# nubot-nudt/LCR-Net

Measured on AMD Instinct MI355X. Metric: scans/s (120k-pt KITTI-shape scan -> 256-D descriptor), higher is better.
Workload: dtype f32 (K-deep GEMMs, K >= 288 and N >= 64: fp32 operands as bf16 x 3 split, 6 of 9 products on the bf16 matrix cores, fp32 accumulate — error vs fp64 <= the fp32-MFMA kernel's; every other GEMM, KPConv and attention: fp32 MFMA); 1 GPU; configs[1]: batch of 8 synthetic 64-beam scans (~120k pts, 0.3 m voxel -> ~16k pts), voxelise + 3 subsamples + 10 radius searches + KPConv encoder + NetVLAD, seeded random weights; distinct_input_batches=4, streams=pre-processing stream (own host thread, 2 batches ahead) + 2 encoder stream(s), parallelism=scan-parallel x1, all-gather of descriptors

## Files before the change

### include/lcr_hip.h

```cpp
#ifndef LCR_HIP_H
#define LCR_HIP_H
#include <stddef.h>
#include <stdint.h>
#ifdef __cplusplus
extern "C" {
#endif

#define LCR_OK 0
#define LCR_EARG (-1)
#define LCR_ESPACE (-2)
#define LCR_EHIP (-3)

#define LCR_STATUS_KEY_OVERFLOW 1u
#define LCR_STATUS_LEN_MISMATCH 2u
#define LCR_GN_REPLICAS 8

const char* lcr_last_error(void);
void lcr_ktimer_enable(int on);
void lcr_ktimer_sample(int every);
void lcr_ktimer_kinds(unsigned mask);
int lcr_ktimer_read(int kind, int max_records, double* seconds, int64_t* meta);
int lcr_ktimer_read2(int kind, int max_records, double* seconds, double* seconds_kernel, int64_t* meta);
int lcr_stream_spin(int microseconds, void* stream);
int lcr_version(void);
// ... 65 lines not shown
  size_t  off_neighbors[LCR_MAX_STAGES];
  size_t  off_subsampling[LCR_MAX_STAGES];
  size_t  off_upsampling[LCR_MAX_STAGES];
  size_t  out_bytes, ws_bytes;
} LcrPrecomputeLayout;
int lcr_precompute_layout(int64_t n0, int B, int num_stages, const int* limits, int upsampling, int64_t n_raw,
                          LcrPrecomputeLayout* layout);
int lcr_precompute_batch(const float* points0, const int64_t* lengths0, const LcrPrecomputeLayout* layout, float voxel_size,
                         float radius, float raw_voxel, int key_bits_hint, void* out, size_t out_bytes, void* ws, size_t ws_bytes,
                         int64_t* lengths_host, uint32_t* status_host, void* stream);
int lcr_precompute_batch_rows(const float* points0, int raw_row_floats, const int64_t* lengths0, const LcrPrecomputeLayout* layout,
                              float voxel_size, float radius, float raw_voxel, int key_bits_hint, void* out, size_t out_bytes, void* ws,
                              size_t ws_bytes, int64_t* lengths_host, uint32_t* status_host, void* stream);
int lcr_precompute_ws_bytes_ex(const LcrPrecomputeLayout* layout, int raw_method, size_t* bytes);
int lcr_precompute_batch_rows_ex(const float* points0, int raw_row_floats, const int64_t* lengths0, const LcrPrecomputeLayout* layout,
                                 float voxel_size, float radius, double raw_voxel, int raw_method, int key_bits_hint, void* out,
                                 size_t out_bytes, void* ws, size_t ws_bytes, int64_t* lengths_host, uint32_t* status_host, void* stream);

int lcr_gemm_f32(const float* A, const float* B, float* C, int64_t M, int N, int K, int transA, int transB,
                 const float* bias, const float* rowdiv, const int64_t* seg_len, int S, int groups, double* stats,
                 void* stream);
int lcr_split_bf16x3(const float* w, int64_t n, uint16_t* planes, void* stream);
int lcr_split_bf16x3_tiles(const float* w, int N, int K, uint16_t* tiles, void* stream);
int lcr_gemm_f32_bsplit(const float* A, const uint16_t* Bs_tiles, float* C, int64_t M, int N, int K, const float* bias, const float* rowdiv,
                        const int64_t* seg_len, int S, int groups, double* stats, void* stream);
int lcr_gemm_f32_masked(const float* A, const float* B, float* C, int64_t M, int N, int K, const float* bias, const float* rowdiv,
                        const int64_t* seg_len, int S, int groups, double* stats, const uint16_t* row_mask, int block_k, void* stream);
int lcr_gemm_f32_bsplit_masked(const float* A, const uint16_t* Bs_tiles, float* C, int64_t M, int N, int K, const float* bias,
                               const float* rowdiv, const int64_t* seg_len, int S, int groups, double* stats, const uint16_t* row_mask,
                               int block_k, void* stream);
int lcr_kpconv_mask_ok(int64_t M, int N, int K, int split);
int lcr_gemm_f32_anorm(const float* A, const float* B, float* C, int64_t M, int N, int K, const float* bias,
                       const double* a_stats, const float* a_gamma, const float* a_beta, int a_groups, float a_eps,
                       float a_slope, const int64_t* seg_len, int S, int groups, double* stats, void* stream);
int lcr_gemm_f32_bsplit_anorm(const float* A, const uint16_t* Bs_tiles, float* C, int64_t M, int N, int K, const float* bias,
                              const double* a_stats, const float* a_gamma, const float* a_beta, int a_groups, float a_eps,
                              float a_slope, const int64_t* seg_len, int S, int groups, double* stats, void* stream);
int lcr_gemm_split_ok(int N, int K);
int lcr_gemm_f32_batched_ta(const float* A, const float* B, float* C, int64_t M, int N, int count, const int* k_host,
                            const int64_t* a_off_host, const int64_t* b_off_host, const int64_t* c_off_host, void* stream);
int lcr_kpconv_aggregate(const float* s_feats, const uint8_t* s_pos, const float* q_pts, const float* s_pts,
                         const void* idx, int idx_is_64, int64_t M, int64_t Ns, int H, int C,
                         const float* kernel_points_host, float sigma, float* A, float* nn,
                         const int32_t* order , void* stream);
#define LCR_KP_VALID_FIRST 1
int lcr_kpconv_aggregate_ex(const float* s_feats, const uint8_t* s_pos, const float* q_pts, const float* s_pts,
                            const void* idx, int idx_is_64, int64_t M, int64_t Ns, int H, int C,
                            const float* kernel_points_host, float sigma, float* A, float* nn,
                            const int32_t* order, int flags, void* stream);
int lcr_kpconv_aggregate_mask(const float* s_feats, const uint8_t* s_pos, const float* q_pts, const float* s_pts,
                              const void* idx, int idx_is_64, int64_t M, int64_t Ns, int H, int C,
                              const float* kernel_points_host, float sigma, float* A, float* nn, uint16_t* mask,
                              const int32_t* order, int flags, void* stream);
int lcr_kpconv_fused(const float* s_feats, const uint8_t* s_pos, const float* q_pts, const float* s_pts, const void* idx,
                     int idx_is_64, int64_t M, int64_t Ns, int H, int C, const float* kernel_points_host, float sigma,
                     const float* W, const float* bias, float* out, const int64_t* seg_len, int S, int groups, double* stats,
                     const int32_t* order, void* stream);
int lcr_kpconv_cin1(const float* s_feats, const float* q_pts, const float* s_pts, const void* idx, int idx_is_64,
                    int64_t M, int64_t Ns, int H, const float* kernel_points_host, float sigma, const float* W,
                    const float* bias, int Cout, float* out, const int32_t* order, void* stream);
int lcr_maxpool(const float* x, const void* idx, int idx_is_64, int64_t M, int64_t Ns, int H, int C, float* out,
                const int32_t* order, void* stream);
int lcr_row_positive(const float* x, int64_t N, int C, uint8_t* pos, void* stream);
int lcr_groupnorm_stats(const float* x, int64_t N, int C, int groups, const int64_t* seg_len, int S, double* stats, void* stream);
int lcr_groupnorm_apply(const float* x, const double* stats, const float* gamma, const float* beta, const float* res,
                        const double* res_stats, const float* res_gamma, const float* res_beta, float* y, int64_t N, int C,
                        int groups, const int64_t* seg_len, int S, float eps, float slope, int act, uint8_t* pos, void* stream);

int lcr_neighbor_transpose_ws_bytes(int64_t M, int H, size_t* bytes);
int lcr_neighbor_transpose(const void* idx, int idx_is_64, int64_t M, int64_t Ns, int H, int32_t* row_start, uint32_t* edges,
                           void* ws, size_t ws_bytes, void* stream);
int lcr_kpconv_aggregate_grad(const float* dA, const float* q_pts, const float* s_pts, const int32_t* row_start, const uint32_t* edges,
                              int64_t M, int64_t Ns, int H, int C, const float* kernel_points_host, float sigma, float* d_s_feats,
                              void* stream);
int lcr_kpconv_cin1_grad_ws_bytes(int64_t M, int Cout, int want_feats, size_t* bytes);
int lcr_kpconv_cin1_grad(const float* d_out, const float* s_feats, const float* q_pts, const float* s_pts, const void* idx, int idx_is_64,
                         const float* nn, const int32_t* row_start, const uint32_t* edges, int64_t M, int64_t Ns, int H,
                         const float* kernel_points_host, float sigma, const float* W, int Cout, float* dW, float* dbias,
                         float* d_s_feats, void* ws, size_t ws_bytes, void* stream);
int lcr_maxpool_grad(const float* d_out, const float* x, const float* pooled, const void* idx, int idx_is_64, const int32_t* row_start,
                     const uint32_t* edges, int64_t M, int64_t Ns, int H, int C, uint8_t* winners, float* d_x, void* stream);
int lcr_kpconv_points_grad_ws_bytes(int64_t M, int H, size_t* bytes);
int lcr_kpconv_points_grad(const float* dA, const float* s_feats, const float* q_pts, const float* s_pts, const void* idx, int idx_is_64,
                           const int32_t* row_start, const uint32_t* edges, int64_t M, int64_t Ns, int H, int C,
                           const float* kernel_points_host, float sigma, float* d_q, float* d_s, void* ws, size_t ws_bytes, void* stream);
int lcr_groupnorm_apply_grad_ws_bytes(int64_t N, int C, int groups, int S, size_t* bytes);
int lcr_groupnorm_apply_grad(const float* x, const double* stats, const float* gamma, const float* y, const float* dy, int64_t N, int C,
                             int groups, const int64_t* seg_len, int S, float eps, float slope, int act, float* dx, float* dgamma,
                             float* dbeta, float* dz, void* ws, size_t ws_bytes, void* stream);

#define LCR_ENC_BLOCKS 10
typedef struct LcrUnaryW {
  const float *w, *b;
  const float *gn_w, *gn_b;
  const uint16_t* w_split;
} LcrUnaryW;
typedef struct LcrBlockW {
  int   cin, cout, strided;
  float sigma;
  const float* kernel_points_host;
  const float *kp_w, *kp_b;
  const float* kp_wt;
  const uint16_t* kp_wt_split;
  const float *normconv_w, *normconv_b;
  LcrUnaryW unary1, unary2, shortcut;
} LcrBlockW;
// ... 265 lines not shown
```

### include/lcr_hip_debug.h

```cpp
#ifndef LCR_HIP_DEBUG_H
#define LCR_HIP_DEBUG_H

#ifdef __cplusplus
extern "C" {
#endif

void lcr_gemm_debug_force_tile(int tile);
void lcr_gemm_debug_deep(int mode);
void lcr_gemm_debug_streamk(int mode);
void lcr_groupnorm_debug_general(int on);
void lcr_kpconv_debug_off64(int on);
void lcr_augment_debug_select_mask(uint32_t mask);

#ifdef __cplusplus
}
#endif
#endif
```

### lcr-net_amd/_lib.py

```python
import ctypes
import os
import re
import types

import torch

_PKG = os.path.dirname(os.path.abspath(__file__))
LIB_PATH = os.path.join(_PKG, "liblcr_hip.so")

_lib = None

HEADERS = [os.path.join(_PKG, "..", "include", h) for h in ("lcr_hip.h", "lcr_hip_debug.h")]
_SCALARS = {"int": ctypes.c_int, "int64_t": ctypes.c_int64, "uint32_t": ctypes.c_uint32, "uint64_t": ctypes.c_uint64, "unsigned": ctypes.c_uint,
            "size_t": ctypes.c_size_t, "float": ctypes.c_float, "double": ctypes.c_double}
_RESULTS = {"int": ctypes.c_int, "void": None, "const char*": ctypes.c_char_p}


def parse_header(text):
    text = re.sub(r"/\*.*?\*/|//[^\n]*", " ", text, flags=re.S)
    text = re.sub(r"^\s*#.*$", "", text, flags=re.M)
    sigs = {}
    for m in re.finditer(r"\b(lcr_\w+)\s*\(", text):
        name = m.group(1)
        head = text[:m.start()]
        res = re.sub(r"\s*\*", "*", " ".join(head[max(head.rfind(c) for c in ";{}") + 1:].split()))
        tail = re.match(r"([^()]*)\)\s*;", text[m.end():])
        if res not in _RESULTS or tail is None:
            raise RuntimeError("%s: cannot parse its prototype (result type %r)" % (name, res))
        args = []
        for p in ([] if tail.group(1).strip() in ("", "void") else tail.group(1).split(",")):
            words = re.sub(r"\bconst\b", " ", p).split()
            ctype = ctypes.c_void_p if "*" in p else _SCALARS.get(" ".join(words[:-1] if len(words) > 1 else words))
            if ctype is None:
                raise RuntimeError("%s: parameter %r has no ctypes mapping" % (name, " ".join(p.split())))
            args.append(ctype)
        sigs[name] = (_RESULTS[res], args)
    return sigs


_RELEASES_GIL = {"lcr_roformer_forward", "lcr_precompute_batch", "lcr_precompute_batch_rows", "lcr_precompute_batch_rows_ex", "lcr_hashmap_bucket_host", "lcr_encoder_forward", "lcr_encoder_forward_ex", "lcr_ktimer_read",
                 "lcr_ktimer_read2", "lcr_hashmap_order_host", "lcr_ransac_sample_host", "lcr_icp_point_to_point", "lcr_icp_point_to_plane", "lcr_netvlad_forward", "lcr_log_sinkhorn", "lcr_log_sinkhorn_ex",
                 "lcr_local_global_registration", "lcr_local_global_registration_ex", "lcr_retrieval_topk", "lcr_stream_spin"}


def build():
    import importlib.util
    spec = importlib.util.spec_from_file_location("_lcr_build", os.path.join(_PKG, "csrc", "build.py"))
    mod = importlib.util.module_from_spec(spec)
    spec.loader.exec_module(mod)
    return mod.build()


_RETURNS_VALUE = {"lcr_version", "lcr_kpconv_mask_ok", "lcr_gemm_split_ok", "lcr_ktimer_read", "lcr_ktimer_read2"}


def __getattr__(name):
    if name == "call":
        lib()
        return call
    raise AttributeError(name)


def _raise_on_rc(rc, fn, args):
    if rc:
        check(rc, fn.__name__)
    return rc


def lib():
    global _lib, call
    if _lib is None:
        if not os.path.exists(LIB_PATH):
            raise RuntimeError(
                "liblcr_hip.so not found at %s — build it with `python lcr-net_amd/csrc/build.py` "
                "(there is no CPU fallback for the lcr-net_amd hot path)" % LIB_PATH)
        sigs = {}
        for header in HEADERS:
            with open(header) as f:
                sigs.update(parse_header(f.read()))
        L = ctypes.CDLL(LIB_PATH)
        K = ctypes.PyDLL(LIB_PATH) if os.environ.get("LCR_CTYPES_KEEP_GIL", "1") != "0" else L
        checked = types.SimpleNamespace()
        for name, (res, args) in sigs.items():
            if not hasattr(L, name):
                continue
            dll = L if name in _RELEASES_GIL else K
            for view, fn in ((L, getattr(dll, name)), (checked, dll[name])):
                fn.restype, fn.argtypes = res, args
                if view is checked and res is ctypes.c_int and name not in _RETURNS_VALUE:
                    fn.errcheck = _raise_on_rc
                setattr(view, name, fn)
        _lib, call = L, checked
    return _lib


def check(rc, what):
    if rc != 0:
        msg = lib().lcr_last_error()
        raise RuntimeError("%s failed (rc=%d): %s" % (what, rc, msg.decode() if msg else ""))


def ptr(t):
    return ctypes.c_void_p(t.data_ptr()) if t is not None else ctypes.c_void_p(0)


def stream_ptr(device=None):
# ... 26 lines not shown
```

### lcr-net_amd/csrc/encoder.hip

```cpp
#include <algorithm>
#include <cstdlib>
#include <cstring>

#include "common.h"

#define TURN(call) ([&]() { LaunchTurn turn_; return (call); }())

namespace lcr {

constexpr float ENC_GN_EPS = 1e-5f;
constexpr float ENC_SLOPE = 0.1f;

struct Arena {
  char*  base;
  size_t off, cap;
  template <typename T>
  T* take(size_t n) {
    const size_t o = off;
    off = align_up(off + n * sizeof(T));
    return (base && off <= cap) ? reinterpret_cast<T*>(base + o) : nullptr;
  }
};

struct StageIO {
  const float*   pts;
  const int64_t* seg;
  const int32_t* order;
  int64_t        n;
  int64_t        min_rows;
};

struct StatsPool {
  double* base;
  size_t  off, cap;
  int     S, groups;
  double* take() {
    const size_t n = static_cast<size_t>(GN_REPLICAS) * S * groups * 2;
    if (off + n > cap) return nullptr;
    double* p = base + off;
    off += n;
    return p;
  }
};

static size_t stats_doubles(int S, int groups) { return static_cast<size_t>(GN_REPLICAS) * S * groups * 2 * 44; }

static int unary_raw(const LcrUnaryW& u, const float* x, int64_t n, int cin, int cout, const StageIO& st, StatsPool& sp, Arena& ws,
                     float** y_out, double** stats_out, hipStream_t s) {
  float* y = ws.take<float>(static_cast<size_t>(n) * cout);
  double* stats = sp.take();
  if (!y || !stats) return LCR_ESPACE;
  const bool split = u.w_split && lcr_gemm_split_ok(cout, cin);
  int rc = split ? TURN(lcr_gemm_f32_bsplit(x, u.w_split, y, n, cout, cin, u.b, nullptr, st.seg, sp.S, sp.groups, stats, s))
                 : TURN(lcr_gemm_f32(x, u.w, y, n, cout, cin, 0, 1, u.b, nullptr, st.seg, sp.S, sp.groups, stats, s));
  *y_out = y;
  *stats_out = stats;
  return rc;
}

static int residual_block(const LcrBlockW& b, const float* s_feats, const StageIO& q, const StageIO& sup, const void* idx, int H,
                          StatsPool& sp, Arena& ws, float* out, unsigned enc_flags, hipStream_t s) {
  const int mid = b.cout / 4, g = sp.groups;
  const int64_t M = q.n, Ns = sup.n;
  int rc;
  const float* x = s_feats;
  uint8_t* pos = ws.take<uint8_t>(static_cast<size_t>(Ns));
  if (!pos) return LCR_ESPACE;
  if (b.unary1.w) {
    float* y1;
    double* st1;
    if ((rc = unary_raw(b.unary1, s_feats, Ns, b.cin, mid, sup, sp, ws, &y1, &st1, s))) return rc;
    float* x1 = ws.take<float>(static_cast<size_t>(Ns) * mid);
    if (!x1) return LCR_ESPACE;
    if ((rc = TURN(lcr_groupnorm_apply(y1, st1, b.unary1.gn_w, b.unary1.gn_b, nullptr, nullptr, nullptr, nullptr, x1, Ns, mid, g, sup.seg, sp.S,
                                  ENC_GN_EPS, ENC_SLOPE, 1, pos, s))))
      return rc;
    x = x1;
  } else if ((rc = TURN(lcr_row_positive(s_feats, Ns, b.cin, pos, s)))) {
    return rc;
  }
  float* A = ws.take<float>(static_cast<size_t>(M) * 15 * mid);
  float* nn = ws.take<float>(static_cast<size_t>(M));
  float* kpo = ws.take<float>(static_cast<size_t>(M) * mid);
  uint16_t* kmask = ws.take<uint16_t>(static_cast<size_t>(M));
  double* stc = sp.take();
  if (!A || !nn || !kpo || !kmask || !stc) return LCR_ESPACE;
  static const bool vf_env_off = getenv("LCR_KP_VALID_FIRST") && atoi(getenv("LCR_KP_VALID_FIRST")) == 0;
  const int vf_flag = ((enc_flags & LCR_ENC_LISTS_VALID_FIRST) && !vf_env_off) ? LCR_KP_VALID_FIRST : 0;
  static const bool fused32 = getenv("LCR_KPCONV_FUSED") != nullptr;
  if (fused32 && mid == 32 && sp.S <= 64) {
    if ((rc = TURN(lcr_kpconv_fused(x, pos, q.pts, sup.pts, idx, 0, M, Ns, H, mid, b.kernel_points_host, b.sigma, b.kp_w, b.kp_b, kpo, q.seg, sp.S, g,
                                    stc, q.order, s))))
      return rc;
  } else {
    const bool split = b.kp_wt_split && mid >= 64;
    if (!((split || b.kp_wt) && lcr_kpconv_mask_ok(M, mid, 15 * mid, split))) kmask = nullptr;
    if ((rc = TURN(lcr_kpconv_aggregate_mask(x, pos, q.pts, sup.pts, idx, 0, M, Ns, H, mid, b.kernel_points_host, b.sigma, A, nn, kmask, q.order, vf_flag,
                                             s))))
      return rc;
    if (split) {
      if ((rc = TURN(kmask ? lcr_gemm_f32_bsplit_masked(A, b.kp_wt_split, kpo, M, mid, 15 * mid, b.kp_b, nn, q.seg, sp.S, g, stc, kmask, mid, s)
                           : lcr_gemm_f32_bsplit(A, b.kp_wt_split, kpo, M, mid, 15 * mid, b.kp_b, nn, q.seg, sp.S, g, stc, s))))
        return rc;
    } else if (kmask) {
      if ((rc = TURN(lcr_gemm_f32_masked(A, b.kp_wt, kpo, M, mid, 15 * mid, b.kp_b, nn, q.seg, sp.S, g, stc, kmask, mid, s)))) return rc;
    } else if ((rc = TURN(b.kp_wt ? lcr_gemm_f32(A, b.kp_wt, kpo, M, mid, 15 * mid, 0, 1, b.kp_b, nn, q.seg, sp.S, g, stc, s)
                                  : lcr_gemm_f32(A, b.kp_w, kpo, M, mid, 15 * mid, 0, 0, b.kp_b, nn, q.seg, sp.S, g, stc, s)))) return rc;
  }
  float* y;
  double* sty;
  static const bool no_anorm = getenv("LCR_NO_NORM_ON_LOAD") != nullptr;
  if (!no_anorm && mid <= 256 && mid % 4 == 0 && b.cout > 32 && q.min_rows >= 64) {
    y = ws.take<float>(static_cast<size_t>(M) * b.cout);
    sty = sp.take();
    if (!y || !sty) return LCR_ESPACE;
    const bool split2 = b.unary2.w_split && lcr_gemm_split_ok(b.cout, mid);
    if ((rc = split2 ? TURN(lcr_gemm_f32_bsplit_anorm(kpo, b.unary2.w_split, y, M, b.cout, mid, b.unary2.b, stc, b.normconv_w, b.normconv_b, g,
                                                      ENC_GN_EPS, ENC_SLOPE, q.seg, sp.S, g, sty, s))
                     : TURN(lcr_gemm_f32_anorm(kpo, b.unary2.w, y, M, b.cout, mid, b.unary2.b, stc, b.normconv_w, b.normconv_b, g, ENC_GN_EPS,
                                               ENC_SLOPE, q.seg, sp.S, g, sty, s))))
      return rc;
  } else {
    float* x2 = ws.take<float>(static_cast<size_t>(M) * mid);
    if (!x2) return LCR_ESPACE;
    if ((rc = TURN(lcr_groupnorm_apply(kpo, stc, b.normconv_w, b.normconv_b, nullptr, nullptr, nullptr, nullptr, x2, M, mid, g, q.seg, sp.S, ENC_GN_EPS,
                                  ENC_SLOPE, 1, nullptr, s))))
      return rc;
    if ((rc = unary_raw(b.unary2, x2, M, mid, b.cout, q, sp, ws, &y, &sty, s))) return rc;
  }
  const float* res = s_feats;
  if (b.strided) {
    float* pooled = ws.take<float>(static_cast<size_t>(M) * b.cin);
    if (!pooled) return LCR_ESPACE;
    if ((rc = TURN(lcr_maxpool(s_feats, idx, 0, M, Ns, H, b.cin, pooled, q.order, s)))) return rc;
    res = pooled;
  }
  const double* str = nullptr;
  if (b.shortcut.w) {
    float* r;
    double* st;
    if ((rc = unary_raw(b.shortcut, res, M, b.cin, b.cout, q, sp, ws, &r, &st, s))) return rc;
    res = r;
    str = st;
  }
  return TURN(lcr_groupnorm_apply(y, sty, b.unary2.gn_w, b.unary2.gn_b, res, str, str ? b.shortcut.gn_w : nullptr, str ? b.shortcut.gn_b : nullptr, out,
                             M, b.cout, g, q.seg, sp.S, ENC_GN_EPS, ENC_SLOPE, 1, nullptr, s));
}

static size_t block_ws_bytes(const LcrBlockW& b, int64_t M, int64_t Ns) {
  Arena a{nullptr, 0, ~size_t(0)};
  const int mid = b.cout / 4;
  a.take<uint8_t>(Ns);
  a.take<float>(static_cast<size_t>(Ns) * mid);
  a.take<float>(static_cast<size_t>(Ns) * mid);
  a.take<float>(static_cast<size_t>(M) * 15 * mid);
  a.take<float>(M);
  a.take<float>(static_cast<size_t>(M) * mid);
  a.take<uint16_t>(static_cast<size_t>(M));
  a.take<float>(static_cast<size_t>(M) * mid);
  a.take<float>(static_cast<size_t>(M) * b.cout);
  a.take<float>(static_cast<size_t>(M) * b.cin);
  a.take<float>(static_cast<size_t>(M) * b.cout);
  return a.off;
}

static const int BLOCK_Q[LCR_ENC_BLOCKS] = {0, 1, 1, 1, 2, 2, 2, 3, 3, 3};
static const int BLOCK_S[LCR_ENC_BLOCKS] = {0, 0, 1, 1, 1, 2, 2, 2, 3, 3};

}

using namespace lcr;

extern "C" int lcr_encoder_ws_bytes(const LcrEncoderW* W, const int64_t* n_host, int S, size_t* bytes) {
  if (!W || !n_host || !bytes || S < 1) return LCR_EARG;
  size_t blk = 0, pp = 0;
  for (int i = 0; i < LCR_ENC_BLOCKS; ++i) {
    blk = std::max(blk, block_ws_bytes(W->blocks[i], n_host[BLOCK_Q[i]], n_host[BLOCK_S[i]]));
    pp = std::max(pp, align_up(sizeof(float) * static_cast<size_t>(n_host[BLOCK_Q[i]]) * W->blocks[i].cout));
  }
  pp = std::max(pp, align_up(sizeof(float) * static_cast<size_t>(n_host[0]) * W->c1_cout * 2));
  *bytes = blk + 2 * pp + align_up(sizeof(double) * stats_doubles(S, W->groups)) + 4096;
  return LCR_OK;
}

extern "C" int lcr_encoder_forward(const LcrEncoderW* W, const float* feats0, const float* const* points, const int32_t* const* neighbors,
                                   const int32_t* const* subsampling, const int32_t* const* order, const int64_t* const* seg_len, int S,
                                   const int64_t* n_host, const int64_t* seg_min_rows_host, const int* limits, float* const* out_feats,
                                   void* ws, size_t ws_bytes, void* stream) {
  return lcr_encoder_forward_ex(W, feats0, points, neighbors, subsampling, order, seg_len, S, n_host, seg_min_rows_host, limits, out_feats, 0u, ws,
                                ws_bytes, stream);
}

extern "C" int lcr_encoder_forward_ex(const LcrEncoderW* W, const float* feats0, const float* const* points, const int32_t* const* neighbors,
                                      const int32_t* const* subsampling, const int32_t* const* order, const int64_t* const* seg_len, int S,
                                      const int64_t* n_host, const int64_t* seg_min_rows_host, const int* limits, float* const* out_feats,
                                      unsigned flags, void* ws, size_t ws_bytes, void* stream) {
  if (!W || !feats0 || !points || !neighbors || !subsampling || !seg_len || !n_host || !limits || !out_feats || !ws || S < 1) {
    set_error("lcr_encoder_forward: bad argument");
    return LCR_EARG;
  }
  size_t need = 0;
  lcr_encoder_ws_bytes(W, n_host, S, &need);
  if (ws_bytes < need) {
    set_error("lcr_encoder_forward: workspace too small (%zu < %zu)", ws_bytes, need);
    return LCR_ESPACE;
  }
  hipStream_t s = static_cast<hipStream_t>(stream);
  StageIO st[4];
  for (int i = 0; i < 4; ++i) st[i] = StageIO{points[i], seg_len[i], order ? order[i] : nullptr, n_host[i], seg_min_rows_host ? seg_min_rows_host[i] : 0};
  Arena top{static_cast<char*>(ws), 0, ws_bytes};
  StatsPool sp{top.take<double>(stats_doubles(S, W->groups)), 0, stats_doubles(S, W->groups), S, W->groups};
  size_t pp = 0;
  for (int i = 0; i < LCR_ENC_BLOCKS; ++i) pp = std::max(pp, sizeof(float) * static_cast<size_t>(n_host[BLOCK_Q[i]]) * W->blocks[i].cout);
  pp = std::max(pp, sizeof(float) * static_cast<size_t>(n_host[0]) * W->c1_cout * 2);
  float* ping = reinterpret_cast<float*>(top.take<char>(pp));
  float* pong = reinterpret_cast<float*>(top.take<char>(pp));
  const size_t scratch0 = top.off;
  if (!sp.base || !ping || !pong) return LCR_ESPACE;
  hipMemsetAsync(sp.base, 0, sizeof(double) * sp.cap, s);

  int rc;
  float* cur;
  {
    const int64_t n0 = n_host[0];
    float* raw = ping;
// ... 31 lines not shown
```

### lcr-net_amd/csrc/kpconv.hip

```cpp
#include <algorithm>
#include <cstdlib>

#include "kpconv.h"

namespace lcr {

typedef float floatx4 __attribute__((ext_vector_type(4)));

template <int V> struct VecOf;
template <> struct VecOf<4> { typedef float4 type; };
template <> struct VecOf<2> { typedef float2 type; };
__device__ __forceinline__ float vget(const float4& v, int i) { return i == 0 ? v.x : i == 1 ? v.y : i == 2 ? v.z : v.w; }
__device__ __forceinline__ float vget(const float2& v, int i) { return i == 0 ? v.x : v.y; }
__device__ __forceinline__ float4 vmake(const float (&a)[4]) { return make_float4(a[0], a[1], a[2], a[3]); }
__device__ __forceinline__ float2 vmake(const float (&a)[2]) { return make_float2(a[0], a[1]); }

template <typename IdxT, int C, bool OFF32, bool MASK = false>
__global__ __launch_bounds__(KP_WAVES * 64) void k_kpconv_aggregate_vec(const float* __restrict__ s_feats, const uint8_t* __restrict__ s_pos,
                                                                        const float* __restrict__ q_pts, const float* __restrict__ s_pts,
                                                                        const IdxT* __restrict__ idx, int64_t M, int64_t Ns, int H, KPoints kp,
                                                                        float sigma, float* __restrict__ A, float* __restrict__ nn,
                                                                        const int32_t* __restrict__ order, int valid_first,
                                                                        uint16_t* __restrict__ mask) {
  constexpr int V = C >= 64 ? 4 : 2;
  constexpr int NL = C / (16 * V);
  constexpr int D = NL == 1 ? 4 : 2;
  typedef typename VecOf<V>::type VecT;
  constexpr int PAD = 4 * D + 4;
  __shared__ __attribute__((aligned(16))) float4 s_rel[KP_WAVES][KP_HMAX + PAD];
  const int lane = threadIdx.x & 63, w = __builtin_amdgcn_readfirstlane(threadIdx.x >> 6);
  const int sub = lane >> 4, col = lane & 15;
  const float inv_sigma = 1.f / sigma;
  LCR_KP_SELECT(kp, col, kx, ky, kz);
  const XcdBand band = xcd_band(M, w, KP_WAVES);
  for (int64_t t = band.begin; t < band.end; t += band.stride) {
    const int64_t m = order ? order[t] : t;
    const float qx = q_pts[3 * m], qy = q_pts[3 * m + 1], qz = q_pts[3 * m + 2];
    int n = 0, cnt = 0;
    for (int h0 = 0; h0 < H; h0 += 64) {
      const int h = h0 + lane;
      bool ok, positive = false;
      uint64_t mk;
      if (OFF32 && sizeof(IdxT) == 4) {
        const uint32_t ju = h < H ? static_cast<uint32_t>(reinterpret_cast<const int32_t*>(idx)[static_cast<uint32_t>(m) * static_cast<uint32_t>(H) + static_cast<uint32_t>(h)])
                                  : static_cast<uint32_t>(Ns);
        ok = ju < static_cast<uint32_t>(Ns);
        mk = wave_ballot(ok);
        if (ok) {
          const int slot = n + mbcnt_lt(mk);
          const float* sp = reinterpret_cast<const float*>(reinterpret_cast<const char*>(s_pts) + ju * 12u);
          s_rel[w][slot] = make_float4(sp[0] - qx, sp[1] - qy, sp[2] - qz, __uint_as_float(ju * static_cast<uint32_t>(C * 4)));
          positive = s_pos[ju] != 0;
        }
      } else {
        int64_t j = Ns;
        if (h < H) j = static_cast<int64_t>(idx[m * H + h]);
        ok = j >= 0 && j < Ns;
        mk = wave_ballot(ok);
        if (ok) {
          const int slot = n + mbcnt_lt(mk);
          s_rel[w][slot] = make_float4(s_pts[3 * j] - qx, s_pts[3 * j + 1] - qy, s_pts[3 * j + 2] - qz,
                                       __uint_as_float(OFF32 ? static_cast<uint32_t>(j) * static_cast<uint32_t>(C * 4) : static_cast<uint32_t>(j)));
          positive = s_pos[j] != 0;
        }
      }
      n += __popcll(mk);
      cnt += __popcll(wave_ballot(positive));
      if (valid_first && mk != ~0ull) break;
    }
    if (lane < PAD) s_rel[w][n + lane] = make_float4(1e6f, 1e6f, 1e6f, __uint_as_float(0u));
    wave_sync();

    floatx4 acc[NL][V];
#pragma unroll
    for (int q = 0; q < NL; ++q)
#pragma unroll
      for (int v = 0; v < V; ++v) acc[q][v] = floatx4{0.f, 0.f, 0.f, 0.f};
    const int steps = (n + 3) >> 2;
    float4 p[D];
    VecT f[D][NL];
    auto fetch = [&](int s, float4& pp, VecT (&ff)[NL]) {
      pp = s_rel[w][4 * s + sub];
      if (OFF32) {
        const uint32_t off = __float_as_uint(pp.w) + static_cast<uint32_t>(V * col * 4);
#pragma unroll
        for (int q = 0; q < NL; ++q) ff[q] = *reinterpret_cast<const VecT*>(reinterpret_cast<const char*>(s_feats) + (off + static_cast<uint32_t>(q * 16 * V * 4)));
      } else {
        const float* r = s_feats + static_cast<int64_t>(__float_as_uint(pp.w)) * C + V * col;
#pragma unroll
        for (int q = 0; q < NL; ++q) ff[q] = *reinterpret_cast<const VecT*>(r + q * 16 * V);
      }
    };
    if (n > 0) {
      auto compute = [&](int s, const float4& pp, const VecT (&ff)[NL]) {
        const float wv = kp_influence(pp.x, pp.y, pp.z, kx, ky, kz, inv_sigma);
#pragma unroll
        for (int q = 0; q < NL; ++q)
#pragma unroll
          for (int v = 0; v < V; ++v) acc[q][v] = __builtin_amdgcn_mfma_f32_16x16x4f32(wv, vget(ff[q], v), acc[q][v], 0, 0, 0);
      };
#pragma unroll
      for (int d = 0; d < D; ++d) fetch(d, p[d], f[d]);
      int s0 = 0;
      for (; s0 + D <= steps; s0 += D) {
#pragma unroll
        for (int d = 0; d < D; ++d) {
          compute(s0 + d, p[d], f[d]);
          fetch(s0 + d + D, p[d], f[d]);
        }
      }
#pragma unroll
      for (int d = 0; d < D - 1; ++d)
        if (s0 + d < steps) compute(s0 + d, p[d], f[d]);
    }
    uint32_t kmask = 0x7fffu;
    if constexpr (MASK) {
      uint32_t bits = 0;
#pragma unroll
      for (int r = 0; r < 4; ++r) {
        uint32_t o = 0;
#pragma unroll
        for (int q = 0; q < NL; ++q)
#pragma unroll
          for (int v = 0; v < V; ++v) o |= __float_as_uint(acc[q][v][r]);
        const uint64_t b = wave_ballot((o & 0x7fffffffu) != 0u);
#pragma unroll
        for (int s4 = 0; s4 < 4; ++s4)
          if ((b >> (16 * s4)) & 0xffffull) bits |= 1u << (4 * s4 + r);
      }
      kmask = bits & 0x7fffu;
      if (lane == 0) mask[m] = static_cast<uint16_t>(kmask);
    }
    float* out = A + m * (KP_K * C) + V * col;
#pragma unroll
    for (int r = 0; r < 4; ++r) {
      const int k = 4 * sub + r;
      if (k < KP_K && ((kmask >> k) & 1u)) {
#pragma unroll
        for (int q = 0; q < NL; ++q) {
          float a[V];
#pragma unroll
          for (int v = 0; v < V; ++v) a[v] = acc[q][v][r];
          *reinterpret_cast<VecT*>(out + k * C + q * 16 * V) = vmake(a);
        }
      }
    }
    if (lane == 0) nn[m] = static_cast<float>(cnt > 1 ? cnt : 1);
    wave_sync();
  }
}

constexpr int KF_C = 32, KF_Q = 16, KF_QW = KF_Q / KP_WAVES, KF_KK = KP_K * KF_C, KF_LD = KF_KK + 4, KF_KW = KF_KK / KP_WAVES;
constexpr int KF_MAX_SEG = 64;

template <typename IdxT>
__global__ __launch_bounds__(KP_WAVES * 64, 3) void k_kpconv_fused32(const float* __restrict__ s_feats, const uint8_t* __restrict__ s_pos,
                                                                     const float* __restrict__ q_pts, const float* __restrict__ s_pts,
                                                                     const IdxT* __restrict__ idx, int64_t M, int64_t Ns, int H, KPoints kp,
                                                                     float sigma, const float* __restrict__ W, const float* __restrict__ bias,
                                                                     float* __restrict__ out, const int64_t* __restrict__ seg_len, int S,
                                                                     int groups, double* __restrict__ stats, const int32_t* __restrict__ order) {
  constexpr int C = KF_C, V = 2, D = 4;
  __shared__ __attribute__((aligned(16))) float s_D[KF_Q * KF_LD];
  __shared__ __attribute__((aligned(16))) float s_P[KP_WAVES][KF_Q][C];
  __shared__ __attribute__((aligned(16))) float4 s_rel[KP_WAVES][KP_HMAX + 8];
  __shared__ int64_t s_m[KF_Q], s_start[KF_MAX_SEG + 1];
// ... 352 lines not shown
      for (int c = lane * 2; c < C; c += 128) {
        float2 v = make_float2(init, init);
        for (int h0 = 0; h0 < n; h0 += 8) {
          float2 f[8];
#pragma unroll
          for (int u = 0; u < 8; ++u)
            f[u] = *reinterpret_cast<const float2*>(x + static_cast<int64_t>(s_idx[w][h0 + u < n ? h0 + u : n - 1]) * C + c);
#pragma unroll
          for (int u = 0; u < 8; ++u) {
            v.x = fmaxf(v.x, f[u].x);
            v.y = fmaxf(v.y, f[u].y);
          }
        }
        *reinterpret_cast<float2*>(out + m * C + c) = v;
      }
    } else {
      for (int c = lane; c < C; c += 64) {
        float v = init;
        for (int h0 = 0; h0 < n; h0 += 8) {
          float f[8];
#pragma unroll
          for (int u = 0; u < 8; ++u) f[u] = x[static_cast<int64_t>(s_idx[w][h0 + u < n ? h0 + u : n - 1]) * C + c];
#pragma unroll
          for (int u = 0; u < 8; ++u) v = fmaxf(v, f[u]);
        }
        out[m * C + c] = v;
      }
    }
    wave_sync();
  }
}

__global__ __launch_bounds__(256) void k_row_pos(const float* __restrict__ x, int64_t N, int C, uint8_t* __restrict__ pos) {
  const int lane = threadIdx.x & 63, w = __builtin_amdgcn_readfirstlane(threadIdx.x >> 6);
  for (int64_t n = static_cast<int64_t>(blockIdx.x) * 4 + w; n < N; n += static_cast<int64_t>(gridDim.x) * 4) {
    float s = 0.f;
    for (int c = lane; c < C; c += 64) s += x[n * C + c];
    s = wave_sum(s);
    if (lane == 0) pos[n] = s > 0.f ? 1 : 0;
  }
}

static int grid_for(int64_t rows, int per_block) { return static_cast<int>(std::min<int64_t>((rows + per_block - 1) / per_block, 256 * 16)); }

static int g_agg_force_off64 = 0;

template <typename IdxT>
static int launch_aggregate(const float* s_feats, const uint8_t* s_pos, const float* q_pts, const float* s_pts, const IdxT* idx, int64_t M,
                            int64_t Ns, int H, int C, const KPoints& kp, float sigma, float* A, float* nn, const int32_t* order, int vf,
                            uint16_t* mask, hipStream_t st) {
  dim3 grid(grid_for_xcd(M, KP_WAVES)), block(KP_WAVES * 64);
  const bool off32 = Ns * C < (int64_t(1) << 30) && M * H < (int64_t(1) << 30) && !g_agg_force_off64;
#define LCR_AGG_M(CC, O32, MK) \
  LCR_LAUNCH_TIMED((k_kpconv_aggregate_vec<IdxT, CC, O32, MK>), grid, block, 0, st, s_feats, s_pos, q_pts, s_pts, idx, M, Ns, H, kp, sigma, A, nn, order, vf, mask)
#define LCR_AGG(CC)                            \
  if (mask) {                                  \
    if (off32) LCR_AGG_M(CC, true, true);      \
    else LCR_AGG_M(CC, false, true);           \
  } else if (off32) LCR_AGG_M(CC, true, false); \
  else LCR_AGG_M(CC, false, false);            \
  break
  switch (C) {
    case 32: LCR_AGG(32);
    case 64: LCR_AGG(64);
    case 128: LCR_AGG(128);
    case 256: LCR_AGG(256);
    default: set_error("lcr_kpconv_aggregate: C must be 32, 64, 128 or 256 (got %d)", C); return LCR_EARG;
  }
#undef LCR_AGG
#undef LCR_AGG_M
  return check_launch("lcr_kpconv_aggregate");
}

}

using namespace lcr;

extern "C" void lcr_kpconv_debug_off64(int on) { g_agg_force_off64 = on; }

extern "C" int lcr_kpconv_aggregate(const float* s_feats, const uint8_t* s_pos, const float* q_pts, const float* s_pts, const void* idx,
                                    int idx_is_64, int64_t M, int64_t Ns, int H, int C, const float* kernel_points_host, float sigma,
                                    float* A, float* nn, const int32_t* order, void* stream) {
  return lcr_kpconv_aggregate_ex(s_feats, s_pos, q_pts, s_pts, idx, idx_is_64, M, Ns, H, C, kernel_points_host, sigma, A, nn, order, 0, stream);
}

extern "C" int lcr_kpconv_aggregate_ex(const float* s_feats, const uint8_t* s_pos, const float* q_pts, const float* s_pts, const void* idx,
                                       int idx_is_64, int64_t M, int64_t Ns, int H, int C, const float* kernel_points_host, float sigma,
                                       float* A, float* nn, const int32_t* order, int flags, void* stream) {
  return lcr_kpconv_aggregate_mask(s_feats, s_pos, q_pts, s_pts, idx, idx_is_64, M, Ns, H, C, kernel_points_host, sigma, A, nn, nullptr, order, flags,
                                   stream);
}

extern "C" int lcr_kpconv_aggregate_mask(const float* s_feats, const uint8_t* s_pos, const float* q_pts, const float* s_pts, const void* idx,
                                         int idx_is_64, int64_t M, int64_t Ns, int H, int C, const float* kernel_points_host, float sigma,
                                         float* A, float* nn, uint16_t* mask, const int32_t* order, int flags, void* stream) {
  if (!s_feats || !s_pos || !q_pts || !s_pts || !idx || !kernel_points_host || !A || !nn || M < 0 || Ns < 0 || H < 1 || H > KP_HMAX ||
      !(sigma > 0.f)) {
    set_error("lcr_kpconv_aggregate: bad argument (H must be in [1,%d])", KP_HMAX);
    return LCR_EARG;
  }
  if (M == 0) return LCR_OK;
  const KPoints kp = load_kp(kernel_points_host);
  hipStream_t st = static_cast<hipStream_t>(stream);
  KernelTimerScope timed(KT_AGGREGATE, st, M, Ns, H, C, idx_is_64 ? 8 : 4);
  const int vf = (flags & LCR_KP_VALID_FIRST) ? 1 : 0;
  return idx_is_64 ? launch_aggregate(s_feats, s_pos, q_pts, s_pts, static_cast<const int64_t*>(idx), M, Ns, H, C, kp, sigma, A, nn, order, vf, mask, st)
                   : launch_aggregate(s_feats, s_pos, q_pts, s_pts, static_cast<const int32_t*>(idx), M, Ns, H, C, kp, sigma, A, nn, order, vf, mask, st);
}

extern "C" int lcr_kpconv_fused(const float* s_feats, const uint8_t* s_pos, const float* q_pts, const float* s_pts, const void* idx,
                                int idx_is_64, int64_t M, int64_t Ns, int H, int C, const float* kernel_points_host, float sigma,
                                const float* W, const float* bias, float* out, const int64_t* seg_len, int S, int groups, double* stats,
                                const int32_t* order, void* stream) {
  if (!s_feats || !s_pos || !q_pts || !s_pts || !idx || !kernel_points_host || !W || !out || M < 0 || Ns < 0 || H < 1 || H > KP_HMAX ||
      !(sigma > 0.f) || C != KF_C) {
    set_error("lcr_kpconv_fused: bad argument (C must be %d, H in [1,%d])", KF_C, KP_HMAX);
    return LCR_EARG;
  }
  if (stats && (!seg_len || S < 1 || S > KF_MAX_SEG || groups < 1 || C % groups != 0)) {
    set_error("lcr_kpconv_fused: statistics need seg_len, 1 <= S <= %d and groups dividing C", KF_MAX_SEG);
    return LCR_EARG;
  }
  if (M == 0) return LCR_OK;
  const KPoints kp = load_kp(kernel_points_host);
  hipStream_t st = static_cast<hipStream_t>(stream);
  KernelTimerScope timed(KT_KPCONV_FUSED, st, M, Ns, H, C, idx_is_64 ? 8 : 4);
  static const int n_cu = [] {
    int dev = 0, cus = 0;
    if (hipGetDevice(&dev) != hipSuccess || hipDeviceGetAttribute(&cus, hipDeviceAttributeMultiprocessorCount, dev) != hipSuccess || cus <= 0)
      cus = 256;
    return cus;
// ... 61 lines not shown
```

### lcr-net_amd/functional.py

```python
import ctypes
import os
import threading

import numpy as np
import torch

from . import _lib

GN_EPS = 1e-5
GN_REPLICAS = 8


class KernelTimer:
    KINDS = {"gemm": 0, "kpconv_aggregate": 1, "radius_query": 2, "attention": 3, "kpconv_fused": 4, "sinkhorn": 5}

    def __init__(self, names):
        self.names = set(names)
        self._cache = None

    def summary(self):
        return {k: [(b, m) for b, _, m in v] for k, v in self.records().items()}

    def records(self):
        if self._cache is None:
# ... 271 lines not shown
    return stats


def groupnorm_apply(x, stats, gamma, beta, groups, seg_len=None, res=None, res_norm=None, slope=0.1, act=True, want_pos=False):
    rs, rg, rb = res_norm if res_norm is not None else (None, None, None)
    if _wants_grad(x, gamma, beta, res, rg, rb):
        out = _GroupNormApplyFn.apply(x, gamma, beta, res, rg, rb, stats, rs, int(groups), seg_len, float(slope), bool(act), bool(want_pos))
        return out if want_pos else out[0]
    return _groupnorm_apply(x, stats, gamma, beta, groups, seg_len, res, res_norm, slope, act, want_pos)


def _groupnorm_apply(x, stats, gamma, beta, groups, seg_len=None, res=None, res_norm=None, slope=0.1, act=True, want_pos=False):
    seg_len = _seg(seg_len, x.shape[0], x.device)
    y = torch.empty_like(x)
    pos = torch.empty((x.shape[0],), dtype=torch.uint8, device=x.device) if want_pos else None
    rs, rg, rb = res_norm if res_norm is not None else (None, None, None)
    _lib.call.lcr_groupnorm_apply(_lib.ptr(x), _lib.ptr(stats), _lib.ptr(gamma), _lib.ptr(beta), _lib.ptr(res), _lib.ptr(rs), _lib.ptr(rg),
                                  _lib.ptr(rb), _lib.ptr(y), x.shape[0], x.shape[1], groups, _lib.ptr(seg_len), seg_len.numel(), GN_EPS, float(slope),
                                  int(act), _lib.ptr(pos), _lib.stream_ptr(x.device))
    return (y, pos) if want_pos else y


def row_positive(x):
    pos = torch.empty((x.shape[0],), dtype=torch.uint8, device=x.device)
    _lib.call.lcr_row_positive(_lib.ptr(x), x.shape[0], x.shape[1], _lib.ptr(pos), _lib.stream_ptr(x.device))
    return pos


def _kp_host(kernel_points):
    kp = np.ascontiguousarray(kernel_points, dtype=np.float32)
    assert kp.shape == (15, 3)
    return kp


def kpconv_aggregate(s_feats, s_pos, q_points, s_points, idx, kernel_points_host, sigma, order=None, emit_mask=False):
    _lib.require_cuda(s_feats, q_points, s_points, idx)
    M, H = idx.shape
    Ns, C = s_feats.shape
    assert idx.is_contiguous() and s_feats.is_contiguous() and q_points.is_contiguous() and s_points.is_contiguous()
    A = torch.empty((M, 15 * C), dtype=torch.float32, device=s_feats.device)
    nn = torch.empty((M,), dtype=torch.float32, device=s_feats.device)
    kp = _kp_host(kernel_points_host)
    if emit_mask:
        mask = torch.empty((M,), dtype=torch.int16, device=s_feats.device)
        _lib.call.lcr_kpconv_aggregate_mask(
            _lib.ptr(s_feats), _lib.ptr(s_pos), _lib.ptr(q_points), _lib.ptr(s_points), _lib.ptr(idx), _idx_args(idx), M, Ns, H, C,
            ctypes.c_void_p(kp.ctypes.data), float(sigma), _lib.ptr(A), _lib.ptr(nn), _lib.ptr(mask), _lib.ptr(order), 0,
            _lib.stream_ptr(s_feats.device))
        return A, nn, mask
    _lib.call.lcr_kpconv_aggregate(
        _lib.ptr(s_feats), _lib.ptr(s_pos), _lib.ptr(q_points), _lib.ptr(s_points), _lib.ptr(idx), _idx_args(idx), M, Ns, H, C,
        ctypes.c_void_p(kp.ctypes.data), float(sigma), _lib.ptr(A), _lib.ptr(nn), _lib.ptr(order), _lib.stream_ptr(s_feats.device))
    return A, nn


KPCONV_FUSED_C = 32


def kpconv_fused(s_feats, s_pos, q_points, s_points, idx, kernel_points_host, sigma, weights, bias, seg_len=None, groups=0, order=None):
    _lib.require_cuda(s_feats, q_points, s_points, idx)
    M, H = idx.shape
    Ns, C = s_feats.shape
    assert C == KPCONV_FUSED_C and tuple(weights.shape) == (15, C, C) and weights.is_contiguous()
    assert idx.is_contiguous() and s_feats.is_contiguous() and q_points.is_contiguous() and s_points.is_contiguous()
    out = torch.empty((M, C), dtype=torch.float32, device=s_feats.device)
    stats, S = None, 0
    if groups:
        seg_len = _seg(seg_len, M, s_feats.device)
        S = seg_len.numel()
        stats = _zero_stats(S, groups, s_feats.device)
    kp = _kp_host(kernel_points_host)
    _lib.call.lcr_kpconv_fused(
        _lib.ptr(s_feats), _lib.ptr(s_pos), _lib.ptr(q_points), _lib.ptr(s_points), _lib.ptr(idx), _idx_args(idx), M, Ns, H, C,
        ctypes.c_void_p(kp.ctypes.data), float(sigma), _lib.ptr(weights), _lib.ptr(bias), _lib.ptr(out),
        _lib.ptr(seg_len) if groups else None, S, int(groups), _lib.ptr(stats), _lib.ptr(order), _lib.stream_ptr(s_feats.device))
    return out, stats


def kpconv_cin1(s_feats, q_points, s_points, idx, kernel_points_host, sigma, weights, bias, order=None):
    M, H = idx.shape
    Ns = s_feats.shape[0]
    Cout = weights.shape[-1]
    out = torch.empty((M, Cout), dtype=torch.float32, device=s_feats.device)
    kp = _kp_host(kernel_points_host)
    _lib.call.lcr_kpconv_cin1(_lib.ptr(s_feats), _lib.ptr(q_points), _lib.ptr(s_points), _lib.ptr(idx), _idx_args(idx), M, Ns, H,
                              ctypes.c_void_p(kp.ctypes.data), float(sigma), _lib.ptr(weights), _lib.ptr(bias), Cout,
                              _lib.ptr(out), _lib.ptr(order), _lib.stream_ptr(s_feats.device))
    return out


def maxpool(x, idx, order=None):
    if _wants_grad(x):
        return _MaxPoolFn.apply(x, idx, order)
    return _maxpool(x, idx, order)


def _maxpool(x, idx, order=None):
    M, H = idx.shape
    out = torch.empty((M, x.shape[1]), dtype=torch.float32, device=x.device)
    _lib.call.lcr_maxpool(_lib.ptr(x), _lib.ptr(idx), _idx_args(idx), M, x.shape[0], H, x.shape[1], _lib.ptr(out),
                          _lib.ptr(order), _lib.stream_ptr(x.device))
    return out


class InvertedList:

# ... 1653 lines not shown
```

Baseline: 3124 scans/s.

## Fuse strided-block max-pool shortcut into the KPConv aggregate gather kernel

For strided encoder blocks, the neighbour gather in the KPConv aggregate kernel now also reads the block-input rows (four times the mid width) and max-folds them into the pooled shortcut. This replaces the separate lcr_maxpool launch and its second walk over the neighbour lists. In exchange the aggregate kernel carries more registers and loads, and its prefetch depth drops to 2 in the pooled variant, which may lower occupancy or overlap. It is on by default, and an env var or debug hook can turn it off.

```diff
diff --git a/include/lcr_hip.h b/include/lcr_hip.h
--- a/include/lcr_hip.h
+++ b/include/lcr_hip.h
@@ -141,6 +141,11 @@
                               const void* idx, int idx_is_64, int64_t M, int64_t Ns, int H, int C,
                               const float* kernel_points_host, float sigma, float* A, float* nn, uint16_t* mask,
                               const int32_t* order, int flags, void* stream);
+int lcr_kpconv_aggregate_mask_pool(const float* s_feats, const uint8_t* s_pos, const float* q_pts, const float* s_pts,
+                                   const void* idx, int idx_is_64, int64_t M, int64_t Ns, int H, int C,
+                                   const float* kernel_points_host, float sigma, float* A, float* nn, uint16_t* mask,
+                                   const int32_t* order, int flags, const float* pool_x, int pool_C, float* pooled, void* stream);
+int lcr_kpconv_pool_ok(int64_t M, int64_t Ns, int H, int C, int pool_C, int idx_is_64);
 int lcr_kpconv_fused(const float* s_feats, const uint8_t* s_pos, const float* q_pts, const float* s_pts, const void* idx,
                      int idx_is_64, int64_t M, int64_t Ns, int H, int C, const float* kernel_points_host, float sigma,
                      const float* W, const float* bias, float* out, const int64_t* seg_len, int S, int groups, double* stats,
diff --git a/include/lcr_hip_debug.h b/include/lcr_hip_debug.h
--- a/include/lcr_hip_debug.h
+++ b/include/lcr_hip_debug.h
@@ -10,6 +10,7 @@
 void lcr_gemm_debug_streamk(int mode);
 void lcr_groupnorm_debug_general(int on);
 void lcr_kpconv_debug_off64(int on);
+void lcr_encoder_debug_pool_fused(int mode);
 void lcr_augment_debug_select_mask(uint32_t mask);
 
 #ifdef __cplusplus
diff --git a/lcr-net_amd/_lib.py b/lcr-net_amd/_lib.py
--- a/lcr-net_amd/_lib.py
+++ b/lcr-net_amd/_lib.py
@@ -51,7 +51,7 @@
     return mod.build()
 
 
-_RETURNS_VALUE = {"lcr_version", "lcr_kpconv_mask_ok", "lcr_gemm_split_ok", "lcr_ktimer_read", "lcr_ktimer_read2"}
+_RETURNS_VALUE = {"lcr_version", "lcr_kpconv_mask_ok", "lcr_kpconv_pool_ok", "lcr_gemm_split_ok", "lcr_ktimer_read", "lcr_ktimer_read2"}
 
 
 def __getattr__(name):
diff --git a/lcr-net_amd/csrc/encoder.hip b/lcr-net_amd/csrc/encoder.hip
--- a/lcr-net_amd/csrc/encoder.hip
+++ b/lcr-net_amd/csrc/encoder.hip
@@ -10,6 +10,8 @@
 
 constexpr float ENC_GN_EPS = 1e-5f;
 constexpr float ENC_SLOPE = 0.1f;
+
+static int g_pool_fused = -1;
 
 struct Arena {
   char*  base;
@@ -84,6 +86,7 @@
   float* kpo = ws.take<float>(static_cast<size_t>(M) * mid);
   uint16_t* kmask = ws.take<uint16_t>(static_cast<size_t>(M));
   double* stc = sp.take();
+  float* pooled = nullptr;
   if (!A || !nn || !kpo || !kmask || !stc) return LCR_ESPACE;
   static const bool vf_env_off = getenv("LCR_KP_VALID_FIRST") && atoi(getenv("LCR_KP_VALID_FIRST")) == 0;
   const int vf_flag = ((enc_flags & LCR_ENC_LISTS_VALID_FIRST) && !vf_env_off) ? LCR_KP_VALID_FIRST : 0;
@@ -95,7 +98,14 @@
   } else {
     const bool split = b.kp_wt_split && mid >= 64;
     if (!((split || b.kp_wt) && lcr_kpconv_mask_ok(M, mid, 15 * mid, split))) kmask = nullptr;
-    if ((rc = TURN(lcr_kpconv_aggregate_mask(x, pos, q.pts, sup.pts, idx, 0, M, Ns, H, mid, b.kernel_points_host, b.sigma, A, nn, kmask, q.order, vf_flag,
+    static const bool pool_env_off = getenv("LCR_KP_POOL_FUSED") && atoi(getenv("LCR_KP_POOL_FUSED")) == 0;
+    if (b.strided && kmask && (g_pool_fused >= 0 ? g_pool_fused != 0 : !pool_env_off) && lcr_kpconv_pool_ok(M, Ns, H, mid, b.cin, 0)) {
+      pooled = ws.take<float>(static_cast<size_t>(M) * b.cin);
+      if (!pooled) return LCR_ESPACE;
+      if ((rc = TURN(lcr_kpconv_aggregate_mask_pool(x, pos, q.pts, sup.pts, idx, 0, M, Ns, H, mid, b.kernel_points_host, b.sigma, A, nn, kmask, q.order,
+                                                    vf_flag, s_feats, b.cin, pooled, s))))
+        return rc;
+    } else if ((rc = TURN(lcr_kpconv_aggregate_mask(x, pos, q.pts, sup.pts, idx, 0, M, Ns, H, mid, b.kernel_points_host, b.sigma, A, nn, kmask, q.order, vf_flag,
                                              s))))
       return rc;
     if (split) {
@@ -130,9 +140,11 @@
   }
   const float* res = s_feats;
   if (b.strided) {
-    float* pooled = ws.take<float>(static_cast<size_t>(M) * b.cin);
-    if (!pooled) return LCR_ESPACE;
-    if ((rc = TURN(lcr_maxpool(s_feats, idx, 0, M, Ns, H, b.cin, pooled, q.order, s)))) return rc;
+    if (!pooled) {
+      pooled = ws.take<float>(static_cast<size_t>(M) * b.cin);
+      if (!pooled) return LCR_ESPACE;
+      if ((rc = TURN(lcr_maxpool(s_feats, idx, 0, M, Ns, H, b.cin, pooled, q.order, s)))) return rc;
+    }
     res = pooled;
   }
   const double* str = nullptr;
@@ -171,6 +183,8 @@
 
 using namespace lcr;
 
+extern "C" void lcr_encoder_debug_pool_fused(int mode) { g_pool_fused = mode; }
+
 extern "C" int lcr_encoder_ws_bytes(const LcrEncoderW* W, const int64_t* n_host, int S, size_t* bytes) {
   if (!W || !n_host || !bytes || S < 1) return LCR_EARG;
   size_t blk = 0, pp = 0;
diff --git a/lcr-net_amd/csrc/kpconv.hip b/lcr-net_amd/csrc/kpconv.hip
--- a/lcr-net_amd/csrc/kpconv.hip
+++ b/lcr-net_amd/csrc/kpconv.hip
@@ -15,17 +15,23 @@
 __device__ __forceinline__ float4 vmake(const float (&a)[4]) { return make_float4(a[0], a[1], a[2], a[3]); }
 __device__ __forceinline__ float2 vmake(const float (&a)[2]) { return make_float2(a[0], a[1]); }
 
-template <typename IdxT, int C, bool OFF32, bool MASK = false>
+template <typename IdxT, int C, bool OFF32, bool MASK = false, int PC = 0>
 __global__ __launch_bounds__(KP_WAVES * 64) void k_kpconv_aggregate_vec(const float* __restrict__ s_feats, const uint8_t* __restrict__ s_pos,
                                                                         const float* __restrict__ q_pts, const float* __restrict__ s_pts,
                                                                         const IdxT* __restrict__ idx, int64_t M, int64_t Ns, int H, KPoints kp,
                                                                         float sigma, float* __restrict__ A, float* __restrict__ nn,
                                                                         const int32_t* __restrict__ order, int valid_first,
-                                                                        uint16_t* __restrict__ mask) {
+                                                                        uint16_t* __restrict__ mask, const float* __restrict__ pool_x,
+                                                                        float* __restrict__ pooled) {
+  constexpr bool POOL = PC > 0;
+  static_assert(!POOL || (OFF32 && sizeof(IdxT) == 4 && PC == 4 * C), "the pooled form: 32-bit lists, pool rows four times the feature rows");
   constexpr int V = C >= 64 ? 4 : 2;
   constexpr int NL = C / (16 * V);
-  constexpr int D = NL == 1 ? 4 : 2;
+  constexpr int D = POOL ? 2 : NL == 1 ? 4 : 2;
   typedef typename VecOf<V>::type VecT;
+  constexpr int PV = PC >= 256 ? 4 : 2;
+  constexpr int PNL = POOL ? PC / (64 * PV) : 1;
+  typedef typename VecOf<PV>::type PoolT;
   constexpr int PAD = 4 * D + 4;
   __shared__ __attribute__((aligned(16))) float4 s_rel[KP_WAVES][KP_HMAX + PAD];
   const int lane = threadIdx.x & 63, w = __builtin_amdgcn_readfirstlane(threadIdx.x >> 6);
@@ -37,6 +43,7 @@
     const int64_t m = order ? order[t] : t;
     const float qx = q_pts[3 * m], qy = q_pts[3 * m + 1], qz = q_pts[3 * m + 2];
     int n = 0, cnt = 0;
+    bool shadow = false;
     for (int h0 = 0; h0 < H; h0 += 64) {
       const int h = h0 + lane;
       bool ok, positive = false;
@@ -46,6 +53,7 @@
                                   : static_cast<uint32_t>(Ns);
         ok = ju < static_cast<uint32_t>(Ns);
         mk = wave_ballot(ok);
+        if constexpr (POOL) shadow |= wave_ballot(h < H && !ok) != 0ull;
         if (ok) {
           const int slot = n + mbcnt_lt(mk);
           const float* sp = reinterpret_cast<const float*>(reinterpret_cast<const char*>(s_pts) + ju * 12u);
@@ -79,6 +87,41 @@
     const int steps = (n + 3) >> 2;
     float4 p[D];
     VecT f[D][NL];
+    PoolT g[POOL ? D : 1][4][PNL];
+    PoolT pv[PNL];
+    uint32_t last_off = 0;
+    if constexpr (POOL) {
+      const float init = shadow ? 0.f : -INFINITY;
+#pragma unroll
+      for (int q = 0; q < PNL; ++q) {
+        float a[PV];
+#pragma unroll
+        for (int v = 0; v < PV; ++v) a[v] = init;
+        pv[q] = vmake(a);
+      }
+      if (n > 0) last_off = __builtin_amdgcn_readfirstlane(__float_as_uint(s_rel[w][n - 1].w));
+    }
+    auto fetch_pool = [&](int s, const float4& pp, PoolT (&gg)[4][PNL]) {
+#pragma unroll
+      for (int u = 0; u < 4; ++u) {
+        const uint32_t e = static_cast<uint32_t>(__builtin_amdgcn_readlane(static_cast<int>(__float_as_uint(pp.w)), 16 * u));
+        const uint32_t off = (4 * s + u < n ? e : last_off) * static_cast<uint32_t>(PC / C) + static_cast<uint32_t>(lane * PV * 4);
+#pragma unroll
+        for (int q = 0; q < PNL; ++q)
+          gg[u][q] = *reinterpret_cast<const PoolT*>(reinterpret_cast<const char*>(pool_x) + (off + static_cast<uint32_t>(q * 64 * PV * 4)));
+      }
+    };
+    auto fold_pool = [&](const PoolT (&gg)[4][PNL]) {
+#pragma unroll
+      for (int u = 0; u < 4; ++u)
+#pragma unroll
+        for (int q = 0; q < PNL; ++q) {
+          float a[PV];
+#pragma unroll
+          for (int v = 0; v < PV; ++v) a[v] = fmaxf(vget(pv[q], v), vget(gg[u][q], v));
+          pv[q] = vmake(a);
+        }
+    };
     auto fetch = [&](int s, float4& pp, VecT (&ff)[NL]) {
       pp = s_rel[w][4 * s + sub];
       if (OFF32) {
@@ -100,18 +143,31 @@
           for (int v = 0; v < V; ++v) acc[q][v] = __builtin_amdgcn_mfma_f32_16x16x4f32(wv, vget(ff[q], v), acc[q][v], 0, 0, 0);
       };
 #pragma unroll
-      for (int d = 0; d < D; ++d) fetch(d, p[d], f[d]);
+      for (int d = 0; d < D; ++d) {
+        fetch(d, p[d], f[d]);
+        if constexpr (POOL) fetch_pool(d, p[d], g[d]);
+      }
       int s0 = 0;
       for (; s0 + D <= steps; s0 += D) {
 #pragma unroll
         for (int d = 0; d < D; ++d) {
           compute(s0 + d, p[d], f[d]);
+          if constexpr (POOL) fold_pool(g[d]);
           fetch(s0 + d + D, p[d], f[d]);
+          if constexpr (POOL) fetch_pool(s0 + d + D, p[d], g[d]);
         }
       }
 #pragma unroll
       for (int d = 0; d < D - 1; ++d)
-        if (s0 + d < steps) compute(s0 + d, p[d], f[d]);
+        if (s0 + d < steps) {
+          compute(s0 + d, p[d], f[d]);
+          if constexpr (POOL) fold_pool(g[d]);
+        }
+    }
+    if constexpr (POOL) {
+      float* po = pooled + m * PC + lane * PV;
+#pragma unroll
+      for (int q = 0; q < PNL; ++q) *reinterpret_cast<PoolT*>(po + q * 64 * PV) = pv[q];
     }
     uint32_t kmask = 0x7fffu;
     if constexpr (MASK) {
@@ -570,7 +626,7 @@
   dim3 grid(grid_for_xcd(M, KP_WAVES)), block(KP_WAVES * 64);
   const bool off32 = Ns * C < (int64_t(1) << 30) && M * H < (int64_t(1) << 30) && !g_agg_force_off64;
 #define LCR_AGG_M(CC, O32, MK) \
-  LCR_LAUNCH_TIMED((k_kpconv_aggregate_vec<IdxT, CC, O32, MK>), grid, block, 0, st, s_feats, s_pos, q_pts, s_pts, idx, M, Ns, H, kp, sigma, A, nn, order, vf, mask)
+  LCR_LAUNCH_TIMED((k_kpconv_aggregate_vec<IdxT, CC, O32, MK>), grid, block, 0, st, s_feats, s_pos, q_pts, s_pts, idx, M, Ns, H, kp, sigma, A, nn, order, vf, mask, nullptr, nullptr)
 #define LCR_AGG(CC)                            \
   if (mask) {                                  \
     if (off32) LCR_AGG_M(CC, true, true);      \
@@ -595,6 +651,42 @@
 using namespace lcr;
 
 extern "C" void lcr_kpconv_debug_off64(int on) { g_agg_force_off64 = on; }
+
+extern "C" int lcr_kpconv_pool_ok(int64_t M, int64_t Ns, int H, int C, int pool_C, int idx_is_64) {
+  if (idx_is_64 || g_agg_force_off64 || M < 0 || Ns < 0 || H < 1 || H > KP_HMAX) return 0;
+  if (!(C == 32 || C == 64 || C == 128) || pool_C != 4 * C) return 0;
+  return Ns * static_cast<int64_t>(pool_C) * 4 < (int64_t(1) << 32) && M * H < (int64_t(1) << 30);
+}
+
+extern "C" int lcr_kpconv_aggregate_mask_pool(const float* s_feats, const uint8_t* s_pos, const float* q_pts, const float* s_pts, const void* idx,
+                                              int idx_is_64, int64_t M, int64_t Ns, int H, int C, const float* kernel_points_host, float sigma,
+                                              float* A, float* nn, uint16_t* mask, const int32_t* order, int flags, const float* pool_x,
+                                              int pool_C, float* pooled, void* stream) {
+  if (!s_feats || !s_pos || !q_pts || !s_pts || !idx || !kernel_points_host || !A || !nn || !mask || !pool_x || !pooled || M < 0 || Ns < 0 ||
+      H < 1 || H > KP_HMAX || !(sigma > 0.f)) {
+    set_error("lcr_kpconv_aggregate_mask_pool: bad argument (H must be in [1,%d]; mask, pool_x and pooled are required)", KP_HMAX);
+    return LCR_EARG;
+  }
+  if (!lcr_kpconv_pool_ok(M, Ns, H, C, pool_C, idx_is_64)) {
+    set_error("lcr_kpconv_aggregate_mask_pool: outside the pooled form (int32 idx, C in {32,64,128}, pool_C = 4 C, Ns * pool_C < 2^30, M * H < 2^30): "
+              "C = %d, pool_C = %d, idx_is_64 = %d — ask lcr_kpconv_pool_ok and run lcr_kpconv_aggregate_mask + lcr_maxpool instead", C, pool_C, idx_is_64);
+    return LCR_EARG;
+  }
+  if (M == 0) return LCR_OK;
+  const KPoints kp = load_kp(kernel_points_host);
+  hipStream_t st = static_cast<hipStream_t>(stream);
+  KernelTimerScope timed(KT_AGGREGATE, st, M, Ns, H, C, 4);
+  const int vf = (flags & LCR_KP_VALID_FIRST) ? 1 : 0;
+  const int32_t* ix = static_cast<const int32_t*>(idx);
+  dim3 grid(grid_for_xcd(M, KP_WAVES)), block(KP_WAVES * 64);
+#define LCR_AGG_POOL(CC) \
+  LCR_LAUNCH_TIMED((k_kpconv_aggregate_vec<int32_t, CC, true, true, 4 * CC>), grid, block, 0, st, s_feats, s_pos, q_pts, s_pts, ix, M, Ns, H, kp, sigma, A, nn, order, vf, mask, pool_x, pooled)
+  if (C == 32) LCR_AGG_POOL(32);
+  else if (C == 64) LCR_AGG_POOL(64);
+  else LCR_AGG_POOL(128);
+#undef LCR_AGG_POOL
+  return check_launch("lcr_kpconv_aggregate_mask_pool");
+}
 
 extern "C" int lcr_kpconv_aggregate(const float* s_feats, const uint8_t* s_pos, const float* q_pts, const float* s_pts, const void* idx,
                                     int idx_is_64, int64_t M, int64_t Ns, int H, int C, const float* kernel_points_host, float sigma,
diff --git a/lcr-net_amd/functional.py b/lcr-net_amd/functional.py
--- a/lcr-net_amd/functional.py
+++ b/lcr-net_amd/functional.py
@@ -347,6 +347,28 @@
         _lib.ptr(s_feats), _lib.ptr(s_pos), _lib.ptr(q_points), _lib.ptr(s_points), _lib.ptr(idx), _idx_args(idx), M, Ns, H, C,
         ctypes.c_void_p(kp.ctypes.data), float(sigma), _lib.ptr(A), _lib.ptr(nn), _lib.ptr(order), _lib.stream_ptr(s_feats.device))
     return A, nn
+
+
+def kpconv_pool_ok(M, Ns, H, C, pool_C, idx_is_64=False):
+    return bool(_lib.lib().lcr_kpconv_pool_ok(int(M), int(Ns), int(H), int(C), int(pool_C), int(bool(idx_is_64))))
+
+
+def kpconv_aggregate_pool(s_feats, s_pos, q_points, s_points, idx, kernel_points_host, sigma, pool_x, order=None, flags=0):
+    _lib.require_cuda(s_feats, q_points, s_points, idx, pool_x)
+    M, H = idx.shape
+    Ns, C = s_feats.shape
+    assert idx.is_contiguous() and s_feats.is_contiguous() and q_points.is_contiguous() and s_points.is_contiguous() and pool_x.is_contiguous()
+    assert pool_x.shape[0] == Ns
+    A = torch.empty((M, 15 * C), dtype=torch.float32, device=s_feats.device)
+    nn = torch.empty((M,), dtype=torch.float32, device=s_feats.device)
+    mask = torch.empty((M,), dtype=torch.int16, device=s_feats.device)
+    pooled = torch.empty((M, pool_x.shape[1]), dtype=torch.float32, device=s_feats.device)
+    kp = _kp_host(kernel_points_host)
+    _lib.call.lcr_kpconv_aggregate_mask_pool(
+        _lib.ptr(s_feats), _lib.ptr(s_pos), _lib.ptr(q_points), _lib.ptr(s_points), _lib.ptr(idx), _idx_args(idx), M, Ns, H, C,
+        ctypes.c_void_p(kp.ctypes.data), float(sigma), _lib.ptr(A), _lib.ptr(nn), _lib.ptr(mask), _lib.ptr(order), int(flags),
+        _lib.ptr(pool_x), pool_x.shape[1], _lib.ptr(pooled), _lib.stream_ptr(s_feats.device))
+    return A, nn, mask, pooled
 
 
 KPCONV_FUSED_C = 32
```

Result: no change. 3144 scans/s, median of 6 (+0.6%).
